# maturk/dn-splatter

Measured on NVIDIA H100. Metric: rendered Mpix/s (fwd+bwd, RGB+depth+normal), higher is better.
Workload: dtype f32

## Files before the change

dn_splatter_b200/csrc/ssim.cu:

```cuda
#include "common.cuh"

namespace {

constexpr int SS_R = 5;
constexpr int SS_T = 16;
constexpr int SS_H = SS_T + 2 * SS_R;
constexpr int SS_P = 28;
constexpr int SS_C = 3;
constexpr int SS_NT = 256;

__constant__ float c_win[11] = {1.028380357e-03f, 7.598758209e-03f, 3.600077331e-02f, 1.093606874e-01f, 2.130055279e-01f,
                                2.660117149e-01f, 2.130055279e-01f, 1.093606874e-01f, 3.600077331e-02f, 7.598758209e-03f,
                                1.028380357e-03f};

__device__ __forceinline__ double warp_sum_f64(double v) {
#pragma unroll
  for (int o = 16; o > 0; o >>= 1) v += __shfl_xor_sync(0xffffffffu, v, o);
  return v;
}

template <bool U8>
__device__ __forceinline__ float ld_gt(const void* img, size_t idx) {
  return U8 ? __fmul_rn((float)((const uint8_t*)img)[idx], 1.0f / 255.0f) : ((const float*)img)[idx];
}

template <int NQ_IN, int NQ_OUT, int NC, typename Make>
__device__ __forceinline__ void hpass(float (*s_in)[SS_C][SS_H][SS_P], float (*s_mid)[SS_C][SS_H][SS_T], int tid, Make make) {
  constexpr int items = NC * SS_H * (SS_T / 2);
  for (int it = tid; it < items; it += SS_NT) {
    const int seg = it % (SS_T / 2), r = (it / (SS_T / 2)) % SS_H, c = it / ((SS_T / 2) * SS_H);
    float in[NQ_IN][12];
#pragma unroll
    for (int q = 0; q < NQ_IN; ++q) {
      const float2* p = reinterpret_cast<const float2*>(&s_in[q][c][r][2 * seg]);
#pragma unroll
      for (int k = 0; k < 6; ++k) { const float2 v = p[k]; in[q][2 * k] = v.x; in[q][2 * k + 1] = v.y; }
    }
    float acc[NQ_OUT][2];
#pragma unroll
    for (int q = 0; q < NQ_OUT; ++q) acc[q][0] = acc[q][1] = 0.f;
#pragma unroll
    for (int k = 0; k < 12; ++k) {
      float v[NQ_OUT];
      float src[NQ_IN];
#pragma unroll
      for (int q = 0; q < NQ_IN; ++q) src[q] = in[q][k];
      make(src, v);
#pragma unroll
      for (int q = 0; q < NQ_OUT; ++q) {
        if (k < 11) acc[q][0] += c_win[k] * v[q];
        if (k > 0) acc[q][1] += c_win[k - 1] * v[q];
      }
    }
#pragma unroll
    for (int q = 0; q < NQ_OUT; ++q) *reinterpret_cast<float2*>(&s_mid[q][c][r][2 * seg]) = make_float2(acc[q][0], acc[q][1]);
  }
}

template <int NQ>
__device__ __forceinline__ void vpass(float (*s_mid)[SS_C][SS_H][SS_T], int c, int col, int g, float out[NQ][4]) {
#pragma unroll
  for (int q = 0; q < NQ; ++q) {
    float v[14];
#pragma unroll
    for (int j = 0; j < 14; ++j) v[j] = s_mid[q][c][4 * g + j][col];
#pragma unroll
    for (int o = 0; o < 4; ++o) {
      float acc = 0.f;
#pragma unroll
      for (int k = 0; k < 11; ++k) acc += c_win[k] * v[o + k];
      out[q][o] = acc;
    }
  }
}

template <bool U8, bool L1, int NC, bool METRIC = false>
__global__ void __launch_bounds__(SS_NT) ssim_fwd_kernel(const float* __restrict__ x, const void* __restrict__ y, int H, int W,
                                                        int C, int c0, float* __restrict__ dmaps, float* __restrict__ sum_out) {
  __shared__ __align__(16) float s_in[2][SS_C][SS_H][SS_P];
  __shared__ __align__(16) float s_mid[5][SS_C][SS_H][SS_T];
  __shared__ float red[SS_NT / 32];
  __shared__ float red_l1[SS_NT / 32];
  const int tid = threadIdx.x;
  constexpr int nc = NC;
  const int i0 = blockIdx.y * SS_T - SS_R, j0 = blockIdx.x * SS_T - SS_R;
  if constexpr (METRIC) {
    const size_t img = (size_t)blockIdx.z * H * W * C;
    x += img;
    y = U8 ? (const void*)((const uint8_t*)y + img) : (const void*)((const float*)y + img);
  }
  for (int e = tid; e < SS_H * SS_H * NC; e += SS_NT) {
    const int c = e % NC, q = (e / NC) % SS_H, r = e / (NC * SS_H);
    const int i = i0 + r, j = j0 + q;
    float xv = 0.f, yv = 0.f;
    if (i >= 0 && i < H && j >= 0 && j < W) {
      const size_t p = ((size_t)i * W + j) * C + c0 + c;
      xv = x[p];
      yv = ld_gt<U8>(y, p);
    }
    s_in[0][c][r][q] = xv;
    s_in[1][c][r][q] = yv;
  }
  __syncthreads();
  hpass<2, 5, NC>(s_in, s_mid, tid, [](const float* s, float* v) {
    v[0] = s[0]; v[1] = s[1]; v[2] = s[0] * s[0]; v[3] = s[1] * s[1]; v[4] = s[0] * s[1];
  });
  __syncthreads();
  float ssum = 0.f, lsum = 0.f;
  if (tid < nc * SS_T * 4) {
    const int col = tid % SS_T, g = (tid / SS_T) % 4, c = tid / (SS_T * 4);
    float f[5][4];
    vpass<5>(s_mid, c, col, g, f);
    const int j = blockIdx.x * SS_T + col;
    const size_t n = (size_t)H * W * C;
#pragma unroll
    for (int o = 0; o < 4; ++o) {
      const int i = blockIdx.y * SS_T + 4 * g + o;
      const bool interior = (i >= SS_R) && (i < H - SS_R) && (j >= SS_R) && (j < W - SS_R);
      float s = 0.f, d_mu = 0.f, d_xx = 0.f, d_xy = 0.f;
      if (interior) {
        const float C1 = 0.0001f, C2 = 0.0009f;
        const float mx = f[0][o], my = f[1][o];
        const float sx = f[2][o] - mx * mx, sy = f[3][o] - my * my, sxy = f[4][o] - mx * my;
        const float A1 = 2.f * mx * my + C1, A2 = 2.f * sxy + C2, B1 = mx * mx + my * my + C1, B2 = sx + sy + C2;
        const float inv = 1.0f / (B1 * B2);
        s = A1 * A2 * inv;
        d_xx = -s / B2;
        d_xy = 2.f * A1 * inv;
        d_mu = 2.f * my * (A2 - A1) * inv - 2.f * mx * s / B1 + 2.f * mx * s / B2;
      }
      if (i < H && j < W) {
        const size_t p = ((size_t)i * W + j) * C + c0 + c;
        if constexpr (METRIC) {
          const float d = s_in[0][c][4 * g + o + SS_R][col + SS_R] - s_in[1][c][4 * g + o + SS_R][col + SS_R];
          lsum += d * d;
        } else {
          dmaps[p] = d_mu; dmaps[n + p] = d_xx; dmaps[2 * n + p] = d_xy;
          if (L1) lsum += fabsf(s_in[0][c][4 * g + o + SS_R][col + SS_R] - s_in[1][c][4 * g + o + SS_R][col + SS_R]);
        }
      }
      ssum += s;
    }
  }
  if constexpr (METRIC) {
    __shared__ double red_d[2][SS_NT / 32];
    const double ds = warp_sum_f64(ssum), dl = warp_sum_f64(lsum);
    if ((tid & 31) == 0) { red_d[0][tid >> 5] = ds; red_d[1][tid >> 5] = dl; }
    __syncthreads();
    if (tid == 0) {
      double t = 0.0, tl = 0.0;
#pragma unroll
      for (int w = 0; w < SS_NT / 32; ++w) { t += red_d[0][w]; tl += red_d[1][w]; }
      double* out = reinterpret_cast<double*>(sum_out) + 2 * blockIdx.z;
      if (t != 0.0) atomicAdd(out, t);
      if (tl != 0.0) atomicAdd(out + 1, tl);
    }
    return;
  }
  ssum = warp_sum(ssum);
  if (L1) lsum = warp_sum(lsum);
  if ((tid & 31) == 0) { red[tid >> 5] = ssum; if (L1) red_l1[tid >> 5] = lsum; }
  __syncthreads();
  if (tid == 0) {
    float t = 0.f, tl = 0.f;
#pragma unroll
    for (int w = 0; w < SS_NT / 32; ++w) { t += red[w]; if (L1) tl += red_l1[w]; }
    if (t != 0.f) atomicAdd(sum_out, t);
    if (L1 && tl != 0.f) atomicAdd(sum_out + 1, tl);
  }
}

__global__ void photometric_finish_kernel(float* out, float lambda, float inv_count_ssim, float inv_count_l1) {
  out[2] = (1.0f - lambda) * (out[1] * inv_count_l1) + lambda * (1.0f - out[0] * inv_count_ssim);
}

template <bool U8, int NC>
__global__ void __launch_bounds__(SS_NT) ssim_bwd_kernel(const float* __restrict__ x, const void* __restrict__ y, int H, int W,
                                                        int C, int c0, const float* __restrict__ dmaps, const float* v_mean,
                                                        float w_ssim, float w_l1, float* __restrict__ v_x) {
  __shared__ __align__(16) float s_in[3][SS_C][SS_H][SS_P];
  __shared__ __align__(16) float s_mid[3][SS_C][SS_H][SS_T];
  const int tid = threadIdx.x;
  constexpr int nc = NC;
  const int i0 = blockIdx.y * SS_T - SS_R, j0 = blockIdx.x * SS_T - SS_R;
  const size_t n = (size_t)H * W * C;
  for (int e = tid; e < SS_H * SS_H * NC; e += SS_NT) {
    const int c = e % NC, q = (e / NC) % SS_H, r = e / (NC * SS_H);
    const int i = i0 + r, j = j0 + q;
    float a = 0.f, b = 0.f, d = 0.f;
    if (i >= 0 && i < H && j >= 0 && j < W) {
      const size_t p = ((size_t)i * W + j) * C + c0 + c;
      a = dmaps[p]; b = dmaps[n + p]; d = dmaps[2 * n + p];
    }
    s_in[0][c][r][q] = a; s_in[1][c][r][q] = b; s_in[2][c][r][q] = d;
  }
  __syncthreads();
  hpass<3, 3, NC>(s_in, s_mid, tid, [](const float* s, float* v) { v[0] = s[0]; v[1] = s[1]; v[2] = s[2]; });
  __syncthreads();
  if (tid < nc * SS_T * 4) {
    const int col = tid % SS_T, g = (tid / SS_T) % 4, c = tid / (SS_T * 4);
    float f[3][4];
    vpass<3>(s_mid, c, col, g, f);
    const int j = blockIdx.x * SS_T + col;
    const float count = (float)(H - 2 * SS_R) * (float)(W - 2 * SS_R) * (float)C;
    const float vm = v_mean ? __ldg(v_mean) : 1.0f;
    const float gsc = vm * w_ssim / count;
    const float gl1 = vm * w_l1 / ((float)H * (float)W * (float)C);
#pragma unroll
    for (int o = 0; o < 4; ++o) {
      const int i = blockIdx.y * SS_T + 4 * g + o;
      if (i < H && j < W) {
        const size_t p = ((size_t)i * W + j) * C + c0 + c;
        const float xv = x[p], yv = ld_gt<U8>(y, p);
        const float d = xv - yv;
        v_x[p] = gsc * (f[0][o] + 2.f * xv * f[1][o] + yv * f[2][o]) + gl1 * ((d > 0.f) ? 1.f : ((d < 0.f) ? -1.f : 0.f));
      }
    }
  }
}

}

template <bool L1>
static int launch_ssim_fwd(const float* pred, const void* gt, int gt_is_u8, int H, int W, int C, float* dmaps, float* out, cudaStream_t s) {
  const dim3 grid((W + SS_T - 1) / SS_T, (H + SS_T - 1) / SS_T, 1);
  for (int c0 = 0; c0 < C; c0 += SS_C) {
    const int nc = C - c0 < SS_C ? C - c0 : SS_C;
#define DNR_SSIM_FWD(U8, NC) ssim_fwd_kernel<U8, L1, NC><<<grid, SS_NT, 0, s>>>(pred, gt, H, W, C, c0, dmaps, out)
    if (gt_is_u8) { if (nc == 3) DNR_SSIM_FWD(true, 3); else if (nc == 2) DNR_SSIM_FWD(true, 2); else DNR_SSIM_FWD(true, 1); }
    else { if (nc == 3) DNR_SSIM_FWD(false, 3); else if (nc == 2) DNR_SSIM_FWD(false, 2); else DNR_SSIM_FWD(false, 1); }
#undef DNR_SSIM_FWD
    DNR_CHECK_LAUNCH();
  }
  return 0;
}

static int launch_ssim_bwd(const float* pred, const void* gt, int gt_is_u8, int H, int W, int C, const float* dmaps, const float* v,
                           float w_ssim, float w_l1, float* v_pred, cudaStream_t s) {
  const dim3 grid((W + SS_T - 1) / SS_T, (H + SS_T - 1) / SS_T, 1);
  for (int c0 = 0; c0 < C; c0 += SS_C) {
    const int nc = C - c0 < SS_C ? C - c0 : SS_C;
#define DNR_SSIM_BWD(U8, NC) ssim_bwd_kernel<U8, NC><<<grid, SS_NT, 0, s>>>(pred, gt, H, W, C, c0, dmaps, v, w_ssim, w_l1, v_pred)
    if (gt_is_u8) { if (nc == 3) DNR_SSIM_BWD(true, 3); else if (nc == 2) DNR_SSIM_BWD(true, 2); else DNR_SSIM_BWD(true, 1); }
    else { if (nc == 3) DNR_SSIM_BWD(false, 3); else if (nc == 2) DNR_SSIM_BWD(false, 2); else DNR_SSIM_BWD(false, 1); }
#undef DNR_SSIM_BWD
    DNR_CHECK_LAUNCH();
  }
  return 0;
}

extern "C" int dnr_rgb_metrics(const float* pred, const void* gt, int32_t gt_is_u8, int32_t B, int32_t H, int32_t W, int32_t C,
                               double* out, void* stream) {
  if (!pred || !gt || !out) return DNR_E_NULL;
  if (B <= 0 || B > 65535 || H <= 2 * SS_R || W <= 2 * SS_R || C <= 0) return DNR_E_SIZE;
  cudaStream_t s = (cudaStream_t)stream;
  DNR_CUDA(cudaMemsetAsync(out, 0, 2 * (size_t)B * sizeof(double), s));
  const dim3 grid((W + SS_T - 1) / SS_T, (H + SS_T - 1) / SS_T, B);
  float* o = reinterpret_cast<float*>(out);
  for (int c0 = 0; c0 < C; c0 += SS_C) {
    const int nc = C - c0 < SS_C ? C - c0 : SS_C;
#define DNR_SSIM_MET(U8, NC) ssim_fwd_kernel<U8, false, NC, true><<<grid, SS_NT, 0, s>>>(pred, gt, H, W, C, c0, nullptr, o)
    if (gt_is_u8) { if (nc == 3) DNR_SSIM_MET(true, 3); else if (nc == 2) DNR_SSIM_MET(true, 2); else DNR_SSIM_MET(true, 1); }
    else { if (nc == 3) DNR_SSIM_MET(false, 3); else if (nc == 2) DNR_SSIM_MET(false, 2); else DNR_SSIM_MET(false, 1); }
#undef DNR_SSIM_MET
    DNR_CHECK_LAUNCH();
  }
  return 0;
}

extern "C" int dnr_ssim_fwd_ex(const float* pred, const void* gt, int32_t gt_is_u8, int32_t H, int32_t W, int32_t C, float* dmaps,
                               float* sum_out, void* stream) {
  if (!pred || !gt || !dmaps || !sum_out) return DNR_E_NULL;
  if (H <= 2 * SS_R || W <= 2 * SS_R || C <= 0) return DNR_E_SIZE;
  cudaStream_t s = (cudaStream_t)stream;
  DNR_CUDA(cudaMemsetAsync(sum_out, 0, sizeof(float), s));
  return launch_ssim_fwd<false>(pred, gt, gt_is_u8, H, W, C, dmaps, sum_out, s);
}

extern "C" int dnr_photometric_fwd(const float* pred, const void* gt, int32_t gt_is_u8, int32_t H, int32_t W, int32_t C,
                                   float ssim_lambda, float* dmaps, float* out, void* stream) {
  if (!pred || !gt || !dmaps || !out) return DNR_E_NULL;
  if (H <= 2 * SS_R || W <= 2 * SS_R || C <= 0) return DNR_E_SIZE;
  cudaStream_t s = (cudaStream_t)stream;
  DNR_CUDA(cudaMemsetAsync(out, 0, 3 * sizeof(float), s));
  if (const int rc = launch_ssim_fwd<true>(pred, gt, gt_is_u8, H, W, C, dmaps, out, s)) return rc;
  photometric_finish_kernel<<<1, 1, 0, s>>>(out, ssim_lambda, 1.0f / ((float)(H - 2 * SS_R) * (float)(W - 2 * SS_R) * (float)C),
                                            1.0f / ((float)H * (float)W * (float)C));
  DNR_CHECK_LAUNCH();
  return 0;
}

extern "C" int dnr_photometric_bwd(const float* pred, const void* gt, int32_t gt_is_u8, int32_t H, int32_t W, int32_t C,
                                   float ssim_lambda, const float* dmaps, const float* v_main, float* v_pred, void* stream) {
  if (!pred || !gt || !dmaps || !v_pred) return DNR_E_NULL;
  if (H <= 2 * SS_R || W <= 2 * SS_R || C <= 0) return DNR_E_SIZE;
  return launch_ssim_bwd(pred, gt, gt_is_u8, H, W, C, dmaps, v_main, -ssim_lambda, 1.0f - ssim_lambda, v_pred, (cudaStream_t)stream);
}

extern "C" int dnr_ssim_bwd_ex(const float* pred, const void* gt, int32_t gt_is_u8, int32_t H, int32_t W, int32_t C,
                               const float* dmaps, const float* v_mean, float* v_pred, void* stream) {
  if (!pred || !gt || !dmaps || !v_pred) return DNR_E_NULL;
  if (H <= 2 * SS_R || W <= 2 * SS_R || C <= 0) return DNR_E_SIZE;
  return launch_ssim_bwd(pred, gt, gt_is_u8, H, W, C, dmaps, v_mean, 1.0f, 0.0f, v_pred, (cudaStream_t)stream);
}

extern "C" int dnr_ssim_fwd(const float* pred, const float* gt, int32_t H, int32_t W, int32_t C, float* dmaps, float* sum_out,
                            void* stream) {
  return dnr_ssim_fwd_ex(pred, gt, 0, H, W, C, dmaps, sum_out, stream);
}

extern "C" int dnr_ssim_bwd(const float* pred, const float* gt, int32_t H, int32_t W, int32_t C, const float* dmaps,
                            const float* v_mean, float* v_pred, void* stream) {
  return dnr_ssim_bwd_ex(pred, gt, 0, H, W, C, dmaps, v_mean, v_pred, stream);
}
```

dn_splatter_b200/regularization_strategy.py:

```python
from __future__ import annotations

import ctypes as C
from abc import abstractmethod
from typing import Optional

import torch
import torch.nn as nn
import torch.nn.functional as F
from torch import Tensor

from . import _lib as L
from .losses import DepthLoss, DepthLossType, NormalLoss, NormalLossType

_FUSED_DEPTH = {DepthLossType.EdgeAwareLogL1: 1, DepthLossType.LogL1: 2, DepthLossType.L1: 3, DepthLossType.MSE: 4}


def _shared_holder(*tensors):
    from .rasterize import raster_holder

    hs = [raster_holder(t) for t in tensors if t is not None]
    if not hs or any(h is None for h in hs) or any(h is not hs[0] for h in hs):
        return None
    return hs[0]


class _FusedDNLoss(torch.autograd.Function):

    @staticmethod
    def forward(ctx, pred_depth, pred_normal, gt_depth, gt_normal, gt_img, depth_type: int, depth_lambda: float,
                depth_tolerance: float, use_normal: bool, holder=None, edge_image=None):
        lib = L.load()
        ref = pred_depth if pred_depth is not None else pred_normal
        if ref.device.type != "cuda":
            raise L.DnrError("DNRegularization: the fused regulariser needs CUDA tensors (no CPU path)")
        if depth_type:
            H, W = pred_depth.shape[0], pred_depth.shape[1]
        else:
            H, W = pred_normal.shape[0], pred_normal.shape[1]
        dev = ref.device

        def prep(t, keep_u8=False):
            if t is None:
                return None
            if keep_u8 and t.dtype == torch.uint8:
                return t.detach().to(device=dev).contiguous()
            return t.detach().to(device=dev, dtype=torch.float32).contiguous()

        pd, pn, gd, gi = prep(pred_depth), prep(pred_normal), prep(gt_depth), prep(gt_img)
        gn = prep(gt_normal, keep_u8=True)
        ei = prep(edge_image, keep_u8=True)
        flags = 0
        if gn is not None and gn.dtype == torch.uint8:
            flags |= L.LOSS_NORMAL_U8
        if ei is not None:
            assert ei.dtype == torch.uint8, "edge_image is the raw uint8 image"
            flags |= L.LOSS_EDGE_FROM_IMAGE | L.LOSS_IMG_U8
        partials = torch.empty(12, dtype=torch.float32, device=dev)
        a = L.DnrArgs()
        a.width, a.height = W, H
        a.depth_loss_type, a.use_normal_loss = int(depth_type), int(bool(use_normal))
        a.depth_lambda, a.depth_tolerance = float(depth_lambda), float(depth_tolerance)
        a.loss_flags = flags
        for k, t in dict(out_depth=pd, out_normal=pn, gt_depth=gd, gt_normal=gn, gt_rgb=gi, gt_image=ei,
                         loss_partials=partials).items():
            setattr(a, k, None if t is None else t.data_ptr())
        L.check(lib.dnr_loss_fwd(C.byref(a), L.stream()), "dnr_loss_fwd")
        ctx.keep = (pd, pn, gd, gn, gi, ei, partials)
        ctx.fwd_stream = torch.cuda.current_stream()
        ctx.cfg = (W, H, int(depth_type), int(bool(use_normal)), float(depth_lambda), float(depth_tolerance), flags)
        ctx.shapes = (None if pred_depth is None else pred_depth.shape, None if pred_normal is None else pred_normal.shape)
        ctx.holder = holder
        return partials[11].clone()

    @staticmethod
    def backward(ctx, v):
        with torch.cuda.stream(ctx.fwd_stream):
            return _FusedDNLoss._backward(ctx, v)

    @staticmethod
    def _backward(ctx, v):
        lib = L.load()
        pd, pn, gd, gn, gi, ei, partials = ctx.keep
        W, H, depth_type, use_normal, lam, tol, flags = ctx.cfg
        v = v.detach().to(torch.float32).contiguous()
        none9 = (None,) * 9
        if ctx.holder is not None:
            from .rasterize import zero_token

            ctx.holder.setdefault("deferred", {})["reg"] = dict(
                depth_type=depth_type, use_normal=use_normal, depth_lambda=lam, depth_tolerance=tol, gt_depth=gd,
                gt_normal=gn if use_normal else None, gt_rgb=gi, edge_image=ei, loss_partials=partials, v=v)
            vd = zero_token(pd.view(ctx.shapes[0])) if (depth_type and ctx.needs_input_grad[0]) else None
            vn = zero_token(pn.view(ctx.shapes[1])) if (use_normal and ctx.needs_input_grad[1]) else None
            return (vd, vn) + none9
        a = L.DnrArgs()
        a.width, a.height = W, H
        a.depth_loss_type, a.use_normal_loss, a.depth_lambda, a.depth_tolerance = depth_type, use_normal, lam, tol
        a.loss_flags = flags
        for k, t in dict(out_depth=pd, out_normal=pn, gt_depth=gd, gt_normal=gn, gt_rgb=gi, gt_image=ei,
                         loss_partials=partials, v_loss=v).items():
            setattr(a, k, None if t is None else t.data_ptr())
        vd = torch.empty(ctx.shapes[0], dtype=torch.float32, device=v.device) if (depth_type and ctx.needs_input_grad[0]) else None
        vn = torch.empty(ctx.shapes[1], dtype=torch.float32, device=v.device) if (use_normal and ctx.needs_input_grad[1]) else None
        if vd is not None or vn is not None:
            L.check(lib.dnr_loss_bwd(C.byref(a), None if vd is None else vd.data_ptr(),
                                     None if vn is None else vn.data_ptr(), L.stream()), "dnr_loss_bwd")
        return (vd, vn) + none9


class _ScaleLoss(torch.autograd.Function):

    @staticmethod
    def forward(ctx, scales):
        lib = L.load()
        if scales.device.type != "cuda":
            raise L.DnrError("scale loss: CUDA tensor required (no CPU path)")
        s = scales.detach().float().contiguous()
        out = torch.empty(1, dtype=torch.float32, device=s.device)
        L.check(lib.dnr_scale_loss_fwd(s.data_ptr(), s.shape[0], out.data_ptr(), L.stream()), "dnr_scale_loss_fwd")
        ctx.s = s
        ctx.fwd_stream = torch.cuda.current_stream()
        return out[0].clone()

    @staticmethod
    def backward(ctx, v):
        with torch.cuda.stream(ctx.fwd_stream):
            return _ScaleLoss._backward(ctx, v)

    @staticmethod
    def _backward(ctx, v):
        lib = L.load()
        s = ctx.s
        v = v.detach().float().contiguous()
        g = torch.empty_like(s)
        L.check(lib.dnr_scale_loss_bwd(s.data_ptr(), s.shape[0], v.data_ptr(), g.data_ptr(), L.stream()),
                "dnr_scale_loss_bwd")
        return g


class FusedL1(torch.autograd.Function):

    @staticmethod
    def forward(ctx, pred, gt, holder=None):
        lib = L.load()
        if pred.device.type != "cuda" or gt.device != pred.device:
            raise L.DnrError("FusedL1 needs CUDA tensors on one device (no CPU path)")
        p = pred.detach().float().contiguous()
        g = gt.detach().contiguous()
        if g.dtype != torch.uint8:
            g = g.float()
        assert g.numel() == p.numel(), "pred / gt size mismatch"
        out = torch.empty(1, dtype=torch.float32, device=p.device)
        L.check(lib.dnr_l1_fwd(p.data_ptr(), g.data_ptr(), p.numel(), int(g.dtype == torch.uint8), out.data_ptr(), L.stream()),
                "dnr_l1_fwd")
        ctx.keep = (p, g)
        ctx.shape = pred.shape
        ctx.fwd_stream = torch.cuda.current_stream()
        ctx.holder = holder
        return out[0].clone()

    @staticmethod
    def backward(ctx, v):
        with torch.cuda.stream(ctx.fwd_stream):
            return FusedL1._backward(ctx, v)

    @staticmethod
    def _backward(ctx, v):
        lib = L.load()
        p, g = ctx.keep
        v = v.detach().float().contiguous()
        if ctx.holder is not None:
            from .rasterize import zero_token

            ctx.holder.setdefault("deferred", {})["l1"] = dict(gt=g, v=v)
            return zero_token(p.view(ctx.shape)), None, None
        vp = torch.empty_like(p)
        L.check(lib.dnr_l1_bwd(p.data_ptr(), g.data_ptr(), p.numel(), int(g.dtype == torch.uint8), v.data_ptr(), vp.data_ptr(),
                               L.stream()), "dnr_l1_bwd")
        return vp.view(ctx.shape), None, None


class FusedSSIM(torch.autograd.Function):

    @staticmethod
    def forward(ctx, pred, gt):
        lib = L.load()
        if pred.device.type != "cuda" or gt.device != pred.device:
            raise L.DnrError("FusedSSIM needs CUDA tensors on one device (no CPU path)")
        p = pred.detach().float().contiguous()
        g = gt.detach().contiguous()
        if g.dtype != torch.uint8:
            g = g.float()
        assert p.dim() == 3 and p.shape == g.shape, "pred / gt must both be [H,W,C]"
        H, W, Cn = p.shape
        dmaps = torch.empty((3, H, W, Cn), dtype=torch.float32, device=p.device)
        out = torch.empty(1, dtype=torch.float32, device=p.device)
        L.check(lib.dnr_ssim_fwd_ex(p.data_ptr(), g.data_ptr(), int(g.dtype == torch.uint8), H, W, Cn, dmaps.data_ptr(),
                                    out.data_ptr(), L.stream()), "dnr_ssim_fwd_ex")
        ctx.keep = (p, g, dmaps)
        ctx.fwd_stream = torch.cuda.current_stream()
        return out[0] / float((H - 10) * (W - 10) * Cn)

    @staticmethod
    def backward(ctx, v):
        with torch.cuda.stream(ctx.fwd_stream):
            lib = L.load()
            p, g, dmaps = ctx.keep
            v = v.detach().float().contiguous()
            vp = torch.empty_like(p)
            H, W, Cn = p.shape
            L.check(lib.dnr_ssim_bwd_ex(p.data_ptr(), g.data_ptr(), int(g.dtype == torch.uint8), H, W, Cn, dmaps.data_ptr(),
                                        v.data_ptr(), vp.data_ptr(), L.stream()), "dnr_ssim_bwd_ex")
            return vp, None


class FusedPhotometric(torch.autograd.Function):

    @staticmethod
    def forward(ctx, pred, gt, ssim_lambda: float):
        lib = L.load()
        if pred.device.type != "cuda" or gt.device != pred.device:
            raise L.DnrError("FusedPhotometric needs CUDA tensors on one device (no CPU path)")
        p = pred.detach().float().contiguous()
        g = gt.detach().contiguous()
        if g.dtype != torch.uint8:
            g = g.float()
        assert p.dim() == 3 and p.shape == g.shape, "pred / gt must both be [H,W,C]"
        H, W, Cn = p.shape
        dmaps = torch.empty((3, H, W, Cn), dtype=torch.float32, device=p.device)
        out = torch.empty(3, dtype=torch.float32, device=p.device)
        L.check(lib.dnr_photometric_fwd(p.data_ptr(), g.data_ptr(), int(g.dtype == torch.uint8), H, W, Cn, float(ssim_lambda),
                                        dmaps.data_ptr(), out.data_ptr(), L.stream()), "dnr_photometric_fwd")
        ctx.keep = (p, g, dmaps)
        ctx.lam = float(ssim_lambda)
        ctx.fwd_stream = torch.cuda.current_stream()
        return out[2].clone()

    @staticmethod
    def backward(ctx, v):
        with torch.cuda.stream(ctx.fwd_stream):
            lib = L.load()
            p, g, dmaps = ctx.keep
            v = v.detach().float().contiguous()
            vp = torch.empty_like(p)
            H, W, Cn = p.shape
            L.check(lib.dnr_photometric_bwd(p.data_ptr(), g.data_ptr(), int(g.dtype == torch.uint8), H, W, Cn, ctx.lam,
                                            dmaps.data_ptr(), v.data_ptr(), vp.data_ptr(), L.stream()), "dnr_photometric_bwd")
            return vp, None, None


def u8_to_float(img: Tensor, divisor: float = 255.0, clamp_min: float = 0.0) -> Tensor:
    src = img.contiguous()
    dst = torch.empty(src.shape, dtype=torch.float32, device=src.device)
    L.check(L.load().dnr_u8_to_f32(src.data_ptr(), src.numel(), float(divisor), float(clamp_min), dst.data_ptr(), L.stream()),
            "dnr_u8_to_f32")
    return dst


class RegularizationStrategy(nn.Module):

    def __init__(self, **kwargs):
        super().__init__()
        self.device_indicator_param = nn.Parameter(torch.empty(0))

    @property
    def device(self):
        return self.device_indicator_param.device

    @abstractmethod
    def get_loss(self, **kwargs):
        """Loss"""

    def forward(self, **kwargs):
        return self.get_loss(**kwargs)

    def get_scale_loss(self, scales):
        return _ScaleLoss.apply(scales)


class DNRegularization(RegularizationStrategy):

    def __init__(self, depth_tolerance: float = 0.1,
                 depth_loss_type: Optional[DepthLossType] = DepthLossType.EdgeAwareLogL1,
                 depth_lambda: float = 0.2, normal_lambda: float = 0.1):
        super().__init__()
        self.depth_tolerance = depth_tolerance
        self.depth_loss_type = depth_loss_type
        self.depth_loss = DepthLoss(self.depth_loss_type)
        self.depth_lambda = depth_lambda
        self.normal_loss_type = NormalLossType.L1
        self.normal_loss = NormalLoss(self.normal_loss_type)
        self.normal_smooth_loss_type = NormalLossType.Smooth
        self.normal_smooth_loss = NormalLoss(self.normal_smooth_loss_type)
        self.normal_lambda = normal_lambda

    def _fusable(self, with_depth: bool) -> bool:
        return (not with_depth) or self.depth_loss_type in _FUSED_DEPTH

    fuse_backward = True
    """Hand the backward of the fused terms to dnr_raster_bwd when the maps are direct raster outputs; DNSplatterModel sets
    it from DNSplatterModelConfig.fuse_loss_backward (False: dnr_loss_bwd writes gradient images)."""

    def get_loss(self, pred_depth, gt_depth, pred_normal, gt_normal, **kwargs):
        with_depth = self.depth_loss is not None
        with_normal = self.normal_loss is not None
        if self._fusable(with_depth) and (with_depth or with_normal):
            if with_depth and gt_depth is None:
                raise TypeError("use_depth_loss is set but the batch holds no depth (reference: '>' on NoneType)")
            dtype = _FUSED_DEPTH[self.depth_loss_type] if with_depth else 0
            gt_img = kwargs.get("gt_img") if dtype == 1 else None
            edge_image = None
            if dtype == 1 and gt_img is None:
                raise KeyError("gt_img")
            if gt_img is not None and gt_img.dtype == torch.uint8:
                gt_img, edge_image = None, gt_img
            pd, pn = (pred_depth if with_depth else None), (pred_normal if with_normal else None)
            holder = _shared_holder(pd, pn) if self.fuse_backward else None
            loss = _FusedDNLoss.apply(pd, pn, gt_depth if with_depth else None, gt_normal if with_normal else None, gt_img,
                                      dtype, self.depth_lambda, self.depth_tolerance, with_normal, holder, edge_image)
        else:
            if gt_normal is not None and gt_normal.dtype == torch.uint8:
                gt_normal = u8_to_float(gt_normal) if gt_normal.is_cuda else gt_normal.float() / 255.0
            if kwargs.get("gt_img") is not None and kwargs["gt_img"].dtype == torch.uint8:
                gi = kwargs["gt_img"]
                kwargs["gt_img"] = u8_to_float(gi, 255.0, 10 / 255.0) if gi.is_cuda else (gi.float() / 255.0).clamp(min=10 / 255.0)
            loss = 0.0
            if with_depth:
                loss = loss + self.get_depth_loss(pred_depth, gt_depth, **kwargs)
            if with_normal:
                loss = loss + self.get_normal_loss(pred_normal, gt_normal, **kwargs)
        return loss + self.get_scale_loss(scales=kwargs["scales"])

    def get_depth_loss(self, pred_depth, gt_depth, **kwargs):
        valid = gt_depth > self.depth_tolerance
        if self.depth_loss_type in _FUSED_DEPTH:
            gt_img = kwargs.get("gt_img") if self.depth_loss_type == DepthLossType.EdgeAwareLogL1 else None
            return _FusedDNLoss.apply(pred_depth, None, gt_depth, None, gt_img, _FUSED_DEPTH[self.depth_loss_type],
                                      self.depth_lambda, self.depth_tolerance, False)
        if self.depth_loss_type == DepthLossType.PearsonDepth:
            n_valid = valid.sum()
            glob = (self.depth_loss(pred_depth, gt_depth.float()) * n_valid) / n_valid
            local = (DepthLoss(DepthLossType.LocalPearsonDepthLoss)(pred_depth, gt_depth.float()) * n_valid) / n_valid
            d = glob + self.depth_lambda * local
            return d + self.depth_lambda * d
        d = self.depth_loss(pred_depth[valid], gt_depth[valid].float())
        return d + self.depth_lambda * d

    def get_normal_loss(self, pred_normal, gt_normal, **kwargs):
        return _FusedDNLoss.apply(None, pred_normal, None, gt_normal, None, 0, 0.0, self.depth_tolerance, True)


def mean_angular_error(pred: Tensor, gt: Tensor) -> Tensor:
    return torch.arccos(torch.clip((gt * pred).sum(0), -1.0, 1.0))


def find_edges(im: Tensor, threshold: float = 0.01, dilation_itr: int = 1) -> Tensor:
    c = im.shape[0]
    lap = torch.tensor([[0, 1, 0], [1, -4, 1], [0, 1, 0]], dtype=torch.float32, device=im.device)
    lap = lap[None, None].expand(c, 1, 3, 3).contiguous()
    box = torch.ones(c, 1, 3, 3, dtype=torch.float32, device=im.device)
    edges = (F.conv2d((1.0 / (im.float() + 1e-6))[None], lap, padding=1, groups=c) > threshold).float()
    dil = edges
    for _ in range(dilation_itr):
        dil = F.conv2d(dil if c == 1 else edges, box, padding=1, groups=c)
    return dil[0] > 0.0


class AGSMeshRegularization(RegularizationStrategy):

    def __init__(self, depth_tolerance: float = 0.1,
                 depth_loss_type: Optional[DepthLossType] = DepthLossType.EdgeAwareLogL1, depth_lambda: float = 0.2,
                 normal_lambda: float = 0.1, normal_mask_steps: int = 15000, depth_mask_steps: int = 7000):
        super().__init__()
        self.depth_tolerance, self.depth_loss_type = depth_tolerance, depth_loss_type
        self.depth_loss = DepthLoss(self.depth_loss_type)
        self.depth_lambda = depth_lambda
        self.normal_loss_type = NormalLossType.L1
        self.normal_loss = NormalLoss(self.normal_loss_type)
        self.normal_smooth_loss_type = NormalLossType.Smooth
        self.normal_smooth_loss = NormalLoss(self.normal_smooth_loss_type)
        self.normal_lambda = normal_lambda
        self.normal_mask_steps, self.depth_mask_steps = normal_mask_steps, depth_mask_steps
        self.step = 0

    def get_loss(self, step, pred_depth, gt_depth, surf_normal, gt_normal, pred_normal, confidence_map, **kwargs):
        d = self.get_depth_loss(step=step, pred_depth=pred_depth, gt_depth=gt_depth, confidence_map=confidence_map, **kwargs)
        n = self.get_normal_loss(step, surf_normal, gt_normal, pred_normal)
        return d + n + self.get_scale_loss(scales=kwargs["scales"])

    def get_scale_loss(self, scales):
        return torch.min(torch.exp(scales), dim=1, keepdim=True)[0].mean()

    def get_depth_loss(self, step, pred_depth, gt_depth, confidence_map, **kwargs):
        if step >= 7000:
            gt_depth = torch.where(confidence_map > 0, gt_depth, torch.zeros_like(gt_depth))
        mask = gt_depth > self.depth_tolerance
        if self.depth_loss_type == DepthLossType.EdgeAwareLogL1:
            return self.depth_loss(pred_depth, gt_depth.float(), kwargs["gt_img"], mask) * self.depth_lambda
        return self.depth_loss(pred_depth[mask], gt_depth[mask]) * self.depth_lambda

    def get_normal_loss(self, step, surf_normal, gt_normal, pred_normal):
        lam = self.normal_lambda if step > 7000 else 0.0
        if step < self.normal_mask_steps:
            keep = ~find_edges(gt_normal)
            l1 = self.normal_loss(surf_normal[keep], gt_normal[keep]) * lam
        else:
            conf = ~(mean_angular_error(surf_normal, gt_normal) > 0.1)
            l1 = self.normal_loss(surf_normal[:, conf], gt_normal[:, conf]) * lam
        return l1 + self.normal_loss(pred_normal, gt_normal) * lam
```

Baseline: 781.6.

## Rewrite SSIM kernels as warp-per-channel sliding row bands with register ring buffers

```diff
diff --git a/dn_splatter_b200/csrc/ssim.cu b/dn_splatter_b200/csrc/ssim.cu
--- a/dn_splatter_b200/csrc/ssim.cu
+++ b/dn_splatter_b200/csrc/ssim.cu
@@ -3,11 +3,12 @@
 namespace {
 
 constexpr int SS_R = 5;
-constexpr int SS_T = 16;
-constexpr int SS_H = SS_T + 2 * SS_R;
-constexpr int SS_P = 28;
+constexpr int SS_K = 2 * SS_R + 1;
+constexpr int SS_TW = 32;
+constexpr int SS_IW = SS_TW + 2 * SS_R;
+constexpr int SS_BAND = 64;
+constexpr int SS_MIN_CTAS = 8;
 constexpr int SS_C = 3;
-constexpr int SS_NT = 256;
 
 __constant__ float c_win[11] = {1.028380357e-03f, 7.598758209e-03f, 3.600077331e-02f, 1.093606874e-01f, 2.130055279e-01f,
                                 2.660117149e-01f, 2.130055279e-01f, 1.093606874e-01f, 3.600077331e-02f, 7.598758209e-03f,
@@ -24,147 +25,133 @@
   return U8 ? __fmul_rn((float)((const uint8_t*)img)[idx], 1.0f / 255.0f) : ((const float*)img)[idx];
 }
 
-template <int NQ_IN, int NQ_OUT, int NC, typename Make>
-__device__ __forceinline__ void hpass(float (*s_in)[SS_C][SS_H][SS_P], float (*s_mid)[SS_C][SS_H][SS_T], int tid, Make make) {
-  constexpr int items = NC * SS_H * (SS_T / 2);
-  for (int it = tid; it < items; it += SS_NT) {
-    const int seg = it % (SS_T / 2), r = (it / (SS_T / 2)) % SS_H, c = it / ((SS_T / 2) * SS_H);
-    float in[NQ_IN][12];
-#pragma unroll
-    for (int q = 0; q < NQ_IN; ++q) {
-      const float2* p = reinterpret_cast<const float2*>(&s_in[q][c][r][2 * seg]);
-#pragma unroll
-      for (int k = 0; k < 6; ++k) { const float2 v = p[k]; in[q][2 * k] = v.x; in[q][2 * k + 1] = v.y; }
-    }
-    float acc[NQ_OUT][2];
-#pragma unroll
-    for (int q = 0; q < NQ_OUT; ++q) acc[q][0] = acc[q][1] = 0.f;
-#pragma unroll
-    for (int k = 0; k < 12; ++k) {
-      float v[NQ_OUT];
-      float src[NQ_IN];
-#pragma unroll
-      for (int q = 0; q < NQ_IN; ++q) src[q] = in[q][k];
-      make(src, v);
-#pragma unroll
-      for (int q = 0; q < NQ_OUT; ++q) {
-        if (k < 11) acc[q][0] += c_win[k] * v[q];
-        if (k > 0) acc[q][1] += c_win[k - 1] * v[q];
-      }
-    }
-#pragma unroll
-    for (int q = 0; q < NQ_OUT; ++q) *reinterpret_cast<float2*>(&s_mid[q][c][r][2 * seg]) = make_float2(acc[q][0], acc[q][1]);
-  }
-}
-
-template <int NQ>
-__device__ __forceinline__ void vpass(float (*s_mid)[SS_C][SS_H][SS_T], int c, int col, int g, float out[NQ][4]) {
-#pragma unroll
-  for (int q = 0; q < NQ; ++q) {
-    float v[14];
-#pragma unroll
-    for (int j = 0; j < 14; ++j) v[j] = s_mid[q][c][4 * g + j][col];
-#pragma unroll
-    for (int o = 0; o < 4; ++o) {
-      float acc = 0.f;
-#pragma unroll
-      for (int k = 0; k < 11; ++k) acc += c_win[k] * v[o + k];
-      out[q][o] = acc;
-    }
-  }
-}
+struct StripLane {
+  int j, ja, jb;
+  bool va, vb;
+  __device__ StripLane(int W) {
+    const int lane = threadIdx.x & 31;
+    j = blockIdx.x * SS_TW + lane;
+    ja = j - SS_R;
+    jb = ja + SS_TW;
+    va = ja >= 0 && ja < W;
+    vb = lane < 2 * SS_R && jb < W;
+  }
+};
 
 template <bool U8, bool L1, int NC, bool METRIC = false>
-__global__ void __launch_bounds__(SS_NT) ssim_fwd_kernel(const float* __restrict__ x, const void* __restrict__ y, int H, int W,
-                                                        int C, int c0, float* __restrict__ dmaps, float* __restrict__ sum_out) {
-  __shared__ __align__(16) float s_in[2][SS_C][SS_H][SS_P];
-  __shared__ __align__(16) float s_mid[5][SS_C][SS_H][SS_T];
-  __shared__ float red[SS_NT / 32];
-  __shared__ float red_l1[SS_NT / 32];
-  const int tid = threadIdx.x;
-  constexpr int nc = NC;
-  const int i0 = blockIdx.y * SS_T - SS_R, j0 = blockIdx.x * SS_T - SS_R;
+__global__ void __launch_bounds__(32 * SS_C, SS_MIN_CTAS)
+    ssim_fwd_kernel(const float* __restrict__ x, const void* __restrict__ y, int H, int W, int C, int c0, int band,
+                    float* __restrict__ dmaps, float* __restrict__ sum_out) {
+  __shared__ float2 s_row[NC][SS_IW];
+  const int lane = threadIdx.x & 31, w = threadIdx.x >> 5, c = c0 + w;
+  const StripLane sl(W);
+  const int i0 = blockIdx.y * band;
+  const int rows = min(band, H - i0);
+  const int n_in = rows + 2 * SS_R;
+  const long long rs = (long long)W * C, oa = (long long)sl.ja * C + c, ob = (long long)sl.jb * C + c;
   if constexpr (METRIC) {
     const size_t img = (size_t)blockIdx.z * H * W * C;
     x += img;
     y = U8 ? (const void*)((const uint8_t*)y + img) : (const void*)((const float*)y + img);
   }
-  for (int e = tid; e < SS_H * SS_H * NC; e += SS_NT) {
-    const int c = e % NC, q = (e / NC) % SS_H, r = e / (NC * SS_H);
-    const int i = i0 + r, j = j0 + q;
-    float xv = 0.f, yv = 0.f;
-    if (i >= 0 && i < H && j >= 0 && j < W) {
-      const size_t p = ((size_t)i * W + j) * C + c0 + c;
-      xv = x[p];
-      yv = ld_gt<U8>(y, p);
-    }
-    s_in[0][c][r][q] = xv;
-    s_in[1][c][r][q] = yv;
-  }
-  __syncthreads();
-  hpass<2, 5, NC>(s_in, s_mid, tid, [](const float* s, float* v) {
-    v[0] = s[0]; v[1] = s[1]; v[2] = s[0] * s[0]; v[3] = s[1] * s[1]; v[4] = s[0] * s[1];
-  });
-  __syncthreads();
+  const size_t n = (size_t)H * W;
+  float2 va, vb;
+  auto load = [&](int r) {
+    va = vb = make_float2(0.f, 0.f);
+    if (r >= 0 && r < H) {
+      const long long row = r * rs;
+      if (sl.va) va = make_float2(x[row + oa], ld_gt<U8>(y, row + oa));
+      if (sl.vb) vb = make_float2(x[row + ob], ld_gt<U8>(y, row + ob));
+    }
+  };
+  float2* sw = s_row[w];
+  float ring[5][SS_K];
   float ssum = 0.f, lsum = 0.f;
-  if (tid < nc * SS_T * 4) {
-    const int col = tid % SS_T, g = (tid / SS_T) % 4, c = tid / (SS_T * 4);
-    float f[5][4];
-    vpass<5>(s_mid, c, col, g, f);
-    const int j = blockIdx.x * SS_T + col;
-    const size_t n = (size_t)H * W * C;
-#pragma unroll
-    for (int o = 0; o < 4; ++o) {
-      const int i = blockIdx.y * SS_T + 4 * g + o;
-      const bool interior = (i >= SS_R) && (i < H - SS_R) && (j >= SS_R) && (j < W - SS_R);
-      float s = 0.f, d_mu = 0.f, d_xx = 0.f, d_xy = 0.f;
-      if (interior) {
-        const float C1 = 0.0001f, C2 = 0.0009f;
-        const float mx = f[0][o], my = f[1][o];
-        const float sx = f[2][o] - mx * mx, sy = f[3][o] - my * my, sxy = f[4][o] - mx * my;
-        const float A1 = 2.f * mx * my + C1, A2 = 2.f * sxy + C2, B1 = mx * mx + my * my + C1, B2 = sx + sy + C2;
-        const float inv = 1.0f / (B1 * B2);
-        s = A1 * A2 * inv;
-        d_xx = -s / B2;
-        d_xy = 2.f * A1 * inv;
-        d_mu = 2.f * my * (A2 - A1) * inv - 2.f * mx * s / B1 + 2.f * mx * s / B2;
-      }
-      if (i < H && j < W) {
-        const size_t p = ((size_t)i * W + j) * C + c0 + c;
-        if constexpr (METRIC) {
-          const float d = s_in[0][c][4 * g + o + SS_R][col + SS_R] - s_in[1][c][4 * g + o + SS_R][col + SS_R];
-          lsum += d * d;
-        } else {
-          dmaps[p] = d_mu; dmaps[n + p] = d_xx; dmaps[2 * n + p] = d_xy;
-          if (L1) lsum += fabsf(s_in[0][c][4 * g + o + SS_R][col + SS_R] - s_in[1][c][4 * g + o + SS_R][col + SS_R]);
-        }
-      }
-      ssum += s;
+  load(i0 - SS_R);
+  for (int t0 = 0; t0 < n_in; t0 += SS_K) {
+#pragma unroll
+    for (int u = 0; u < SS_K; ++u) {
+      const int t = t0 + u;
+      if (t >= n_in) break;
+      __syncwarp();
+      sw[lane] = va;
+      if (lane < 2 * SS_R) sw[SS_TW + lane] = vb;
+      __syncwarp();
+      if (t + 1 < n_in) load(i0 - SS_R + t + 1);
+      float acc[5] = {0.f, 0.f, 0.f, 0.f, 0.f};
+#pragma unroll
+      for (int k = 0; k < SS_K; ++k) {
+        const float2 in = sw[lane + k];
+        const float xs = in.x, ys = in.y;
+        const float v[5] = {xs, ys, xs * xs, ys * ys, xs * ys};
+#pragma unroll
+        for (int q = 0; q < 5; ++q) acc[q] += c_win[k] * v[q];
+      }
+#pragma unroll
+      for (int q = 0; q < 5; ++q) ring[q][u] = acc[q];
+      if (t >= SS_R && t < SS_R + rows && sl.j < W) {
+        const float2 in = sw[lane + SS_R];
+        const float d = in.x - in.y;
+        if constexpr (METRIC) lsum += d * d;
+        else if (L1) lsum += fabsf(d);
+      }
+      if (t >= 2 * SS_R) {
+        float f[5];
+#pragma unroll
+        for (int q = 0; q < 5; ++q) {
+          float a = 0.f;
+#pragma unroll
+          for (int k = 0; k < SS_K; ++k) a += c_win[k] * ring[q][(u + 1 + k) % SS_K];
+          f[q] = a;
+        }
+        const int i = i0 + t - 2 * SS_R, j = sl.j;
+        const bool interior = (i >= SS_R) && (i < H - SS_R) && (j >= SS_R) && (j < W - SS_R);
+        float s = 0.f, d_mu = 0.f, d_xx = 0.f, d_xy = 0.f;
+        if (interior) {
+          const float C1 = 0.0001f, C2 = 0.0009f;
+          const float mx = f[0], my = f[1];
+          const float sx = f[2] - mx * mx, sy = f[3] - my * my, sxy = f[4] - mx * my;
+          const float A1 = 2.f * mx * my + C1, A2 = 2.f * sxy + C2, B1 = mx * mx + my * my + C1, B2 = sx + sy + C2;
+          const float inv = 1.0f / (B1 * B2);
+          s = A1 * A2 * inv;
+          d_xx = -s / B2;
+          d_xy = 2.f * A1 * inv;
+          d_mu = 2.f * my * (A2 - A1) * inv - 2.f * mx * s / B1 + 2.f * mx * s / B2;
+        }
+        if constexpr (!METRIC) {
+          if (j < W) {
+            const size_t p = (size_t)c * n + (size_t)i * W + j, plane = (size_t)C * n;
+            dmaps[p] = d_mu; dmaps[plane + p] = d_xx; dmaps[2 * plane + p] = d_xy;
+          }
+        }
+        ssum += s;
+      }
     }
   }
   if constexpr (METRIC) {
-    __shared__ double red_d[2][SS_NT / 32];
+    __shared__ double red_d[2][SS_C];
     const double ds = warp_sum_f64(ssum), dl = warp_sum_f64(lsum);
-    if ((tid & 31) == 0) { red_d[0][tid >> 5] = ds; red_d[1][tid >> 5] = dl; }
+    if (lane == 0) { red_d[0][w] = ds; red_d[1][w] = dl; }
     __syncthreads();
-    if (tid == 0) {
+    if (threadIdx.x == 0) {
       double t = 0.0, tl = 0.0;
 #pragma unroll
-      for (int w = 0; w < SS_NT / 32; ++w) { t += red_d[0][w]; tl += red_d[1][w]; }
+      for (int v = 0; v < NC; ++v) { t += red_d[0][v]; tl += red_d[1][v]; }
       double* out = reinterpret_cast<double*>(sum_out) + 2 * blockIdx.z;
       if (t != 0.0) atomicAdd(out, t);
       if (tl != 0.0) atomicAdd(out + 1, tl);
     }
     return;
   }
+  __shared__ float red[2][SS_C];
   ssum = warp_sum(ssum);
   if (L1) lsum = warp_sum(lsum);
-  if ((tid & 31) == 0) { red[tid >> 5] = ssum; if (L1) red_l1[tid >> 5] = lsum; }
+  if (lane == 0) { red[0][w] = ssum; red[1][w] = lsum; }
   __syncthreads();
-  if (tid == 0) {
+  if (threadIdx.x == 0) {
     float t = 0.f, tl = 0.f;
 #pragma unroll
-    for (int w = 0; w < SS_NT / 32; ++w) { t += red[w]; if (L1) tl += red_l1[w]; }
+    for (int v = 0; v < NC; ++v) { t += red[0][v]; if (L1) tl += red[1][v]; }
     if (t != 0.f) atomicAdd(sum_out, t);
     if (L1 && tl != 0.f) atomicAdd(sum_out + 1, tl);
   }
@@ -175,45 +162,78 @@
 }
 
 template <bool U8, int NC>
-__global__ void __launch_bounds__(SS_NT) ssim_bwd_kernel(const float* __restrict__ x, const void* __restrict__ y, int H, int W,
-                                                        int C, int c0, const float* __restrict__ dmaps, const float* v_mean,
-                                                        float w_ssim, float w_l1, float* __restrict__ v_x) {
-  __shared__ __align__(16) float s_in[3][SS_C][SS_H][SS_P];
-  __shared__ __align__(16) float s_mid[3][SS_C][SS_H][SS_T];
-  const int tid = threadIdx.x;
-  constexpr int nc = NC;
-  const int i0 = blockIdx.y * SS_T - SS_R, j0 = blockIdx.x * SS_T - SS_R;
-  const size_t n = (size_t)H * W * C;
-  for (int e = tid; e < SS_H * SS_H * NC; e += SS_NT) {
-    const int c = e % NC, q = (e / NC) % SS_H, r = e / (NC * SS_H);
-    const int i = i0 + r, j = j0 + q;
-    float a = 0.f, b = 0.f, d = 0.f;
-    if (i >= 0 && i < H && j >= 0 && j < W) {
-      const size_t p = ((size_t)i * W + j) * C + c0 + c;
-      a = dmaps[p]; b = dmaps[n + p]; d = dmaps[2 * n + p];
-    }
-    s_in[0][c][r][q] = a; s_in[1][c][r][q] = b; s_in[2][c][r][q] = d;
-  }
-  __syncthreads();
-  hpass<3, 3, NC>(s_in, s_mid, tid, [](const float* s, float* v) { v[0] = s[0]; v[1] = s[1]; v[2] = s[2]; });
-  __syncthreads();
-  if (tid < nc * SS_T * 4) {
-    const int col = tid % SS_T, g = (tid / SS_T) % 4, c = tid / (SS_T * 4);
-    float f[3][4];
-    vpass<3>(s_mid, c, col, g, f);
-    const int j = blockIdx.x * SS_T + col;
-    const float count = (float)(H - 2 * SS_R) * (float)(W - 2 * SS_R) * (float)C;
-    const float vm = v_mean ? __ldg(v_mean) : 1.0f;
-    const float gsc = vm * w_ssim / count;
-    const float gl1 = vm * w_l1 / ((float)H * (float)W * (float)C);
-#pragma unroll
-    for (int o = 0; o < 4; ++o) {
-      const int i = blockIdx.y * SS_T + 4 * g + o;
-      if (i < H && j < W) {
-        const size_t p = ((size_t)i * W + j) * C + c0 + c;
-        const float xv = x[p], yv = ld_gt<U8>(y, p);
-        const float d = xv - yv;
-        v_x[p] = gsc * (f[0][o] + 2.f * xv * f[1][o] + yv * f[2][o]) + gl1 * ((d > 0.f) ? 1.f : ((d < 0.f) ? -1.f : 0.f));
+__global__ void __launch_bounds__(32 * SS_C, SS_MIN_CTAS)
+    ssim_bwd_kernel(const float* __restrict__ x, const void* __restrict__ y, int H, int W, int C, int c0, int band,
+                    const float* __restrict__ dmaps, const float* v_mean, float w_ssim, float w_l1, float* __restrict__ v_x) {
+  __shared__ float s_row[NC][3][SS_IW];
+  const int lane = threadIdx.x & 31, w = threadIdx.x >> 5, c = c0 + w;
+  const StripLane sl(W);
+  const int i0 = blockIdx.y * band;
+  const int rows = min(band, H - i0);
+  const int n_in = rows + 2 * SS_R;
+  const size_t n = (size_t)H * W;
+  const float* maps[3] = {dmaps + (size_t)c * n, dmaps + ((size_t)C + c) * n, dmaps + ((size_t)2 * C + c) * n};
+  float ma[3], mb[3];
+  auto load = [&](int r) {
+#pragma unroll
+    for (int q = 0; q < 3; ++q) ma[q] = mb[q] = 0.f;
+    if (r >= 0 && r < H) {
+      const size_t row = (size_t)r * W;
+#pragma unroll
+      for (int q = 0; q < 3; ++q) {
+        if (sl.va) ma[q] = maps[q][row + sl.ja];
+        if (sl.vb) mb[q] = maps[q][row + sl.jb];
+      }
+    }
+  };
+  const float count = (float)(H - 2 * SS_R) * (float)(W - 2 * SS_R) * (float)C;
+  const float vm = v_mean ? __ldg(v_mean) : 1.0f;
+  const float gsc = vm * w_ssim / count;
+  const float gl1 = vm * w_l1 / ((float)H * (float)W * (float)C);
+  float ring[3][SS_K];
+  load(i0 - SS_R);
+  for (int t0 = 0; t0 < n_in; t0 += SS_K) {
+#pragma unroll
+    for (int u = 0; u < SS_K; ++u) {
+      const int t = t0 + u;
+      if (t >= n_in) break;
+      const int i = i0 + t - 2 * SS_R, j = sl.j;
+      const bool emit = t >= 2 * SS_R && j < W;
+      float xv = 0.f, yv = 0.f;
+      size_t p = 0;
+      if (emit) {
+        p = ((size_t)i * W + j) * C + c;
+        xv = x[p];
+        yv = ld_gt<U8>(y, p);
+      }
+      __syncwarp();
+#pragma unroll
+      for (int q = 0; q < 3; ++q) {
+        s_row[w][q][lane] = ma[q];
+        if (lane < 2 * SS_R) s_row[w][q][SS_TW + lane] = mb[q];
+      }
+      __syncwarp();
+      if (t + 1 < n_in) load(i0 - SS_R + t + 1);
+#pragma unroll
+      for (int q = 0; q < 3; ++q) {
+        float a = 0.f;
+#pragma unroll
+        for (int k = 0; k < SS_K; ++k) a += c_win[k] * s_row[w][q][lane + k];
+        ring[q][u] = a;
+      }
+      if (t >= 2 * SS_R) {
+        float f[3];
+#pragma unroll
+        for (int q = 0; q < 3; ++q) {
+          float a = 0.f;
+#pragma unroll
+          for (int k = 0; k < SS_K; ++k) a += c_win[k] * ring[q][(u + 1 + k) % SS_K];
+          f[q] = a;
+        }
+        if (emit) {
+          const float d = xv - yv;
+          v_x[p] = gsc * (f[0] + 2.f * xv * f[1] + yv * f[2]) + gl1 * ((d > 0.f) ? 1.f : ((d < 0.f) ? -1.f : 0.f));
+        }
       }
     }
   }
@@ -223,10 +243,10 @@
 
 template <bool L1>
 static int launch_ssim_fwd(const float* pred, const void* gt, int gt_is_u8, int H, int W, int C, float* dmaps, float* out, cudaStream_t s) {
-  const dim3 grid((W + SS_T - 1) / SS_T, (H + SS_T - 1) / SS_T, 1);
+  const dim3 grid((W + SS_TW - 1) / SS_TW, (H + SS_BAND - 1) / SS_BAND, 1);
   for (int c0 = 0; c0 < C; c0 += SS_C) {
     const int nc = C - c0 < SS_C ? C - c0 : SS_C;
-#define DNR_SSIM_FWD(U8, NC) ssim_fwd_kernel<U8, L1, NC><<<grid, SS_NT, 0, s>>>(pred, gt, H, W, C, c0, dmaps, out)
+#define DNR_SSIM_FWD(U8, NC) ssim_fwd_kernel<U8, L1, NC><<<grid, 32 * NC, 0, s>>>(pred, gt, H, W, C, c0, SS_BAND, dmaps, out)
     if (gt_is_u8) { if (nc == 3) DNR_SSIM_FWD(true, 3); else if (nc == 2) DNR_SSIM_FWD(true, 2); else DNR_SSIM_FWD(true, 1); }
     else { if (nc == 3) DNR_SSIM_FWD(false, 3); else if (nc == 2) DNR_SSIM_FWD(false, 2); else DNR_SSIM_FWD(false, 1); }
 #undef DNR_SSIM_FWD
@@ -237,10 +257,11 @@
 
 static int launch_ssim_bwd(const float* pred, const void* gt, int gt_is_u8, int H, int W, int C, const float* dmaps, const float* v,
                            float w_ssim, float w_l1, float* v_pred, cudaStream_t s) {
-  const dim3 grid((W + SS_T - 1) / SS_T, (H + SS_T - 1) / SS_T, 1);
+  const dim3 grid((W + SS_TW - 1) / SS_TW, (H + SS_BAND - 1) / SS_BAND, 1);
   for (int c0 = 0; c0 < C; c0 += SS_C) {
     const int nc = C - c0 < SS_C ? C - c0 : SS_C;
-#define DNR_SSIM_BWD(U8, NC) ssim_bwd_kernel<U8, NC><<<grid, SS_NT, 0, s>>>(pred, gt, H, W, C, c0, dmaps, v, w_ssim, w_l1, v_pred)
+#define DNR_SSIM_BWD(U8, NC) ssim_bwd_kernel<U8, NC><<<grid, 32 * NC, 0, s>>>(pred, gt, H, W, C, c0, SS_BAND, dmaps, v, w_ssim, w_l1, \
+                                                                              v_pred)
     if (gt_is_u8) { if (nc == 3) DNR_SSIM_BWD(true, 3); else if (nc == 2) DNR_SSIM_BWD(true, 2); else DNR_SSIM_BWD(true, 1); }
     else { if (nc == 3) DNR_SSIM_BWD(false, 3); else if (nc == 2) DNR_SSIM_BWD(false, 2); else DNR_SSIM_BWD(false, 1); }
 #undef DNR_SSIM_BWD
@@ -255,11 +276,11 @@
   if (B <= 0 || B > 65535 || H <= 2 * SS_R || W <= 2 * SS_R || C <= 0) return DNR_E_SIZE;
   cudaStream_t s = (cudaStream_t)stream;
   DNR_CUDA(cudaMemsetAsync(out, 0, 2 * (size_t)B * sizeof(double), s));
-  const dim3 grid((W + SS_T - 1) / SS_T, (H + SS_T - 1) / SS_T, B);
+  const dim3 grid((W + SS_TW - 1) / SS_TW, (H + SS_BAND - 1) / SS_BAND, B);
   float* o = reinterpret_cast<float*>(out);
   for (int c0 = 0; c0 < C; c0 += SS_C) {
     const int nc = C - c0 < SS_C ? C - c0 : SS_C;
-#define DNR_SSIM_MET(U8, NC) ssim_fwd_kernel<U8, false, NC, true><<<grid, SS_NT, 0, s>>>(pred, gt, H, W, C, c0, nullptr, o)
+#define DNR_SSIM_MET(U8, NC) ssim_fwd_kernel<U8, false, NC, true><<<grid, 32 * NC, 0, s>>>(pred, gt, H, W, C, c0, SS_BAND, nullptr, o)
     if (gt_is_u8) { if (nc == 3) DNR_SSIM_MET(true, 3); else if (nc == 2) DNR_SSIM_MET(true, 2); else DNR_SSIM_MET(true, 1); }
     else { if (nc == 3) DNR_SSIM_MET(false, 3); else if (nc == 2) DNR_SSIM_MET(false, 2); else DNR_SSIM_MET(false, 1); }
 #undef DNR_SSIM_MET
diff --git a/dn_splatter_b200/regularization_strategy.py b/dn_splatter_b200/regularization_strategy.py
--- a/dn_splatter_b200/regularization_strategy.py
+++ b/dn_splatter_b200/regularization_strategy.py
@@ -11,6 +11,7 @@
 
 from . import _lib as L
 from .losses import DepthLoss, DepthLossType, NormalLoss, NormalLossType
+from .rasterize import _timed
 
 _FUSED_DEPTH = {DepthLossType.EdgeAwareLogL1: 1, DepthLossType.LogL1: 2, DepthLossType.L1: 3, DepthLossType.MSE: 4}
 
@@ -64,7 +65,7 @@
         for k, t in dict(out_depth=pd, out_normal=pn, gt_depth=gd, gt_normal=gn, gt_rgb=gi, gt_image=ei,
                          loss_partials=partials).items():
             setattr(a, k, None if t is None else t.data_ptr())
-        L.check(lib.dnr_loss_fwd(C.byref(a), L.stream()), "dnr_loss_fwd")
+        L.check(_timed("loss_fwd", lib.dnr_loss_fwd, C.byref(a), L.stream()), "dnr_loss_fwd")
         ctx.keep = (pd, pn, gd, gn, gi, ei, partials)
         ctx.fwd_stream = torch.cuda.current_stream()
         ctx.cfg = (W, H, int(depth_type), int(bool(use_normal)), float(depth_lambda), float(depth_tolerance), flags)
@@ -117,7 +118,8 @@
             raise L.DnrError("scale loss: CUDA tensor required (no CPU path)")
         s = scales.detach().float().contiguous()
         out = torch.empty(1, dtype=torch.float32, device=s.device)
-        L.check(lib.dnr_scale_loss_fwd(s.data_ptr(), s.shape[0], out.data_ptr(), L.stream()), "dnr_scale_loss_fwd")
+        L.check(_timed("scale_loss_fwd", lib.dnr_scale_loss_fwd, s.data_ptr(), s.shape[0], out.data_ptr(), L.stream()),
+                "dnr_scale_loss_fwd")
         ctx.s = s
         ctx.fwd_stream = torch.cuda.current_stream()
         return out[0].clone()
@@ -133,8 +135,8 @@
         s = ctx.s
         v = v.detach().float().contiguous()
         g = torch.empty_like(s)
-        L.check(lib.dnr_scale_loss_bwd(s.data_ptr(), s.shape[0], v.data_ptr(), g.data_ptr(), L.stream()),
-                "dnr_scale_loss_bwd")
+        L.check(_timed("scale_loss_bwd", lib.dnr_scale_loss_bwd, s.data_ptr(), s.shape[0], v.data_ptr(), g.data_ptr(),
+                       L.stream()), "dnr_scale_loss_bwd")
         return g
 
 
@@ -229,8 +231,8 @@
         H, W, Cn = p.shape
         dmaps = torch.empty((3, H, W, Cn), dtype=torch.float32, device=p.device)
         out = torch.empty(3, dtype=torch.float32, device=p.device)
-        L.check(lib.dnr_photometric_fwd(p.data_ptr(), g.data_ptr(), int(g.dtype == torch.uint8), H, W, Cn, float(ssim_lambda),
-                                        dmaps.data_ptr(), out.data_ptr(), L.stream()), "dnr_photometric_fwd")
+        L.check(_timed("photometric_fwd", lib.dnr_photometric_fwd, p.data_ptr(), g.data_ptr(), int(g.dtype == torch.uint8), H, W,
+                       Cn, float(ssim_lambda), dmaps.data_ptr(), out.data_ptr(), L.stream()), "dnr_photometric_fwd")
         ctx.keep = (p, g, dmaps)
         ctx.lam = float(ssim_lambda)
         ctx.fwd_stream = torch.cuda.current_stream()
@@ -244,8 +246,8 @@
             v = v.detach().float().contiguous()
             vp = torch.empty_like(p)
             H, W, Cn = p.shape
-            L.check(lib.dnr_photometric_bwd(p.data_ptr(), g.data_ptr(), int(g.dtype == torch.uint8), H, W, Cn, ctx.lam,
-                                            dmaps.data_ptr(), v.data_ptr(), vp.data_ptr(), L.stream()), "dnr_photometric_bwd")
+            L.check(_timed("photometric_bwd", lib.dnr_photometric_bwd, p.data_ptr(), g.data_ptr(), int(g.dtype == torch.uint8), H,
+                           W, Cn, ctx.lam, dmaps.data_ptr(), v.data_ptr(), vp.data_ptr(), L.stream()), "dnr_photometric_bwd")
             return vp, None, None
 
 
```

Result: faster. 810.8, median of 6 (+3.7%).
